# 0xSameer/ast

Measured on AMD Instinct MI355X. Metric: speech frames/s (train step), higher is better.
Workload: dtype f32 storage / f32 accumulate; batched GEMMs as bf16x3 splits on the bf16 MFMA pipe (every f32 operand value represented EXACTLY by three bf16 terms, f32 exponent range, six term products, each product exact to 2^-26: >= float32 on any data); the encoder recurrences multiply the same way (resident we

## Files before the change

### ast_amd/_lib.py

```python
import ctypes as C
import os

_HERE = os.path.dirname(os.path.abspath(__file__))
LIB_PATH = os.environ.get("ASTK_LIB_PATH") or os.path.join(_HERE, "libastk.so")

TEST_LIB_PATH = os.path.join(_HERE, "libastk_test.so")

MAX_CNN = 4
MAX_RNN = 8
MAX_ATTN = 4
PREC_DEFAULT, PREC_FP16X2, PREC_BF16X3, PREC_F32 = 0, 1, 2, 3
OPERANDS_DEFAULT, OPERANDS_F32, OPERANDS_FP16 = 0, 1, 2
OPERANDS_BY_NAME = {None: OPERANDS_DEFAULT, "default": OPERANDS_DEFAULT, "f32": OPERANDS_F32, "fp16": OPERANDS_FP16}
PREC_BY_NAME = {None: PREC_DEFAULT, "default": PREC_DEFAULT, "fp16x2": PREC_FP16X2, "bf16x3": PREC_BF16X3, "f32": PREC_F32}

c_float_p = C.POINTER(C.c_float)
c_int_p = C.POINTER(C.c_int32)
c_double_p = C.POINTER(C.c_double)


class _Sized:

    def __init__(self, *a, **k):
        super().__init__()
# ... 172 lines not shown
    "astk_persist_status_snapshot": (C.c_int, [_VP, _VP]),
    "astk_persist_status_merge": (C.c_int, [_VP, _VP]),
    "astk_persist_status": (C.c_int, [C.POINTER(C.c_uint), _I]),
    "astk_device_cu_count": (C.c_int, []),
    "astk_lstm_stack_path": (C.c_int, [C.POINTER(LstmStackDesc)]),
    "astk_lstm_stack_free_cus": (C.c_int, [C.POINTER(LstmStackDesc)]),
    "astk_decoder_path": (C.c_int, [C.POINTER(DecoderDesc)]),
    "astk_prof_begin": (C.c_int, []),
    "astk_prof_end": (C.c_int, [C.POINTER(C.c_double)]),
}

TEST_HOOK_SIGNATURES = {
    "astk_debug_set_amax_generation": (C.c_int, [C.c_uint]),
    "astk_conv_debug_preact": (C.c_int, [C.POINTER(CnnDesc), _VP, _SZ, _I, _VP, _VP]),
    "astk_conv_debug_kill_units": (C.c_int, [_VP, _I]),
    "astk_debug_gemm_group": (C.c_int, [_I, _I, c_int_p, c_int_p, c_int_p, C.POINTER(C.c_void_p), C.POINTER(C.c_void_p), C.POINTER(C.c_void_p), _I, _I, _VP]),
}

_lib = None
_test_lib = None


class AstkError(RuntimeError):
    pass


def load():
    global _lib
    if _lib is not None:
        return _lib
# ... 74 lines not shown
```

### ast_amd/csrc/common.h

```cpp
#pragma once
#include <hip/hip_runtime.h>
#include <stdint.h>
#include <stddef.h>
#include <stdio.h>
#include <string.h>
#include "../../include/astk.h"

namespace astk {

void set_error(const char* fmt, ...);

enum ProfCat { PROF_ATTN_FWD = 0, PROF_ATTN_BWD = 1, PROF_GEMM = 2, PROF_CELL = 3, PROF_DEC_FWD = 4, PROF_DEC_BWD = 5, PROF_NCAT = 6 };
bool prof_enabled();
float* prof_tick_buffer(int which);
void prof_start(int cat, hipStream_t s, double work);
void prof_stop(int cat, hipStream_t s);
void prof_add_bytes(int cat, double bytes);
struct ProfScope {
  int cat; hipStream_t s; bool on;
  ProfScope(int c, hipStream_t st, double work = 0.0) : cat(c), s(st), on(prof_enabled()) { if (on) prof_start(cat, s, work); }
  ~ProfScope() { if (on) prof_stop(cat, s); }
};

#define ASTK_CHECK(cond, ...)            \
// ... 36 lines not shown
enum PersistBit { PERSIST_ENC_FWD = 1, PERSIST_ENC_BWD = 2, PERSIST_DEC_FWD = 4, PERSIST_DEC_BWD = 8 };
struct AbortCtl {
  unsigned* word;
  unsigned* status;
  unsigned limit;
  unsigned bit;
};
AbortCtl abort_ctl(unsigned* word, unsigned bit);
int device_cu_count();
enum TuneKey {
  TUNE_GEMM_TILE, TUNE_GEMM_T256_ABOVE, TUNE_GEMM_GRID, TUNE_GEMM_HYBRID, TUNE_GEMM_CHUNK, TUNE_GEMM_CHUNK_DIV, TUNE_GEMM_LOG, TUNE_GEMM_TICKET,
  TUNE_GEMM_DETERMINISTIC, TUNE_GEMM_FORWARD_PAIRS,
  TUNE_CONV_DIRECT0, TUNE_CONV_SEQ_FWD, TUNE_CONV_SEQ_BWD, TUNE_CONV_SEQ_STATS_BLOCKS, TUNE_CONV_SEQ_APPLY_BLOCKS,
  TUNE_DEC_PERSIST, TUNE_DEC_B6_SPLIT, TUNE_DEC_B6_FUSED, TUNE_DEC_WIDE,
  TUNE_LSTM_PERSIST, TUNE_LSTM_HOIST, TUNE_LSTM_X3, TUNE_LSTM_X4, TUNE_LSTM_ROWS32, TUNE_LSTM_OVERLAP_CHUNK, TUNE_LSTM_SIDE_FWD, TUNE_LSTM_SIDE_BWD, TUNE_LSTM_DUO_SIDE,
  TUNE_ROW_LONGK, TUNE_PERSIST_SPIN_LIMIT, TUNE_COLREDUCE_BLOCKS,
  TUNE_COUNT
};
double tune(TuneKey k);
inline bool tune_on(TuneKey k) { return tune(k) != 0.0; }
__device__ __forceinline__ bool abort_seen(const AbortCtl& ab) {
  return __hip_atomic_load(ab.word, __ATOMIC_RELAXED, __HIP_MEMORY_SCOPE_AGENT) != 0;
}
__device__ __forceinline__ void abort_raise(const AbortCtl& ab) {
  __hip_atomic_store(ab.word, 1u, __ATOMIC_RELAXED, __HIP_MEMORY_SCOPE_AGENT);
  __hip_atomic_fetch_or(ab.status, ab.bit, __ATOMIC_RELAXED, __HIP_MEMORY_SCOPE_AGENT);
}

constexpr int AMAX_SLOT_WORDS = 16;
constexpr int AMAX_PSLOT_STRIDE = 16;
constexpr int AMAX_PSLOT_WORDS = AMAX_SLOT_WORDS * AMAX_PSLOT_STRIDE;
// ... 442 lines not shown
```

### ast_amd/csrc/conv.hip

```cpp
#include "common.h"
#include <atomic>
#include <mutex>
#include <algorithm>
#include <cstdlib>

namespace astk {

namespace {

struct CnnPlan {
  int n;
  int B, T, D;
  int Tn[ASTK_MAX_CNN_LAYERS], Fn[ASTK_MAX_CNN_LAYERS];
  int Tc[ASTK_MAX_CNN_LAYERS], Fc[ASTK_MAX_CNN_LAYERS];
  int pwt[ASTK_MAX_CNN_LAYERS], pwf[ASTK_MAX_CNN_LAYERS];
  bool pooled[ASTK_MAX_CNN_LAYERS];
  int Cn[ASTK_MAX_CNN_LAYERS];
  int rows[ASTK_MAX_CNN_LAYERS];
  int rowsc[ASTK_MAX_CNN_LAYERS];
  int K0, K0p;
  int JG, K0g, xf_rows;
  float* XF;
  int padA[ASTK_MAX_CNN_LAYERS];
  int dF[ASTK_MAX_CNN_LAYERS], dB[ASTK_MAX_CNN_LAYERS];
// ... 375 lines not shown
        }
        if (c + 16 < C) {
          *reinterpret_cast<float4*>(row + c + 16) = make_float4(sa[4], sa[5], sa[6], sa[7]);
          *reinterpret_cast<float4*>(row + C + c + 16) = make_float4(qa[4], qa[5], qa[6], qa[7]);
        }
      }
    }
  }
}
struct UnpackJobs {
  int n;
  const float* src[ASTK_MAX_CNN_LAYERS];
  float* dW[ASTK_MAX_CNN_LAYERS];
  int Co[ASTK_MAX_CNN_LAYERS], Ci[ASTK_MAX_CNN_LAYERS], KT[ASTK_MAX_CNN_LAYERS];
  int JG[ASTK_MAX_CNN_LAYERS], ldg[ASTK_MAX_CNN_LAYERS];
};
__global__ void k_unpack_dw(UnpackJobs jobs, const unsigned* __restrict__ status, float* __restrict__ status_dst) {
  const int q = blockIdx.y;
  if (status_dst && blockIdx.x == 0 && q == 0 && threadIdx.x == 0) *status_dst = (float)(*status);
  const float* const src = jobs.src[q];
  float* const dW = jobs.dW[q];
  const int Co = jobs.Co[q], Ci = jobs.Ci[q], KT = jobs.KT[q], JG = jobs.JG[q], ldg = jobs.ldg[q];
  const long n = (long)Co * Ci * KT;
  for (long i = blockIdx.x * (long)blockDim.x + threadIdx.x; i < n; i += (long)gridDim.x * blockDim.x) {
    if (ldg > 0) {
      const int j = (int)(i % Ci), t = (int)((i / Ci) % KT), c = (int)(i / ((long)Ci * KT));
      dW[i] += src[(long)c * ldg + t * JG + j];
    } else {
      const int k = (int)(i % KT), ci = (int)((i / KT) % Ci), co = (int)(i / ((long)Ci * KT));
      dW[i] += src[((long)co * KT + k) * Ci + ci];
    }
  }
}

__global__ __launch_bounds__(256) void k_repack_w(const float* __restrict__ W, float* __restrict__ Wr, int Co, int Ci, int KT, unsigned long long* amax,
                                                  const unsigned long long* fold_src, unsigned long long* fold_dst) {
  __shared__ float red4[4];
  if (fold_src && blockIdx.x == 0 && threadIdx.x < 64) amax_compact(fold_src, fold_dst);
  const long n = (long)Co * Ci * KT;
  float m = 0.f;
  for (long i = blockIdx.x * (long)blockDim.x + threadIdx.x; i < n; i += (long)gridDim.x * blockDim.x) {
    const int ci = (int)(i % Ci);
    const int k = (int)((i / Ci) % KT);
    const int co = (int)(i / ((long)Ci * KT));
    const float v = W[((long)co * Ci + ci) * KT + k];
    Wr[i] = v;
    m = fmaxf(m, fabsf(v));
  }
  if (amax) amax_emit_block(amax, m, red4);
}
struct PhaseWJobs {
  int n;
  float* wd[GEMM_GROUP_MAX];
  int r[GEMM_GROUP_MAX], na[GEMM_GROUP_MAX];
  unsigned long long* amax[GEMM_GROUP_MAX];
};
__global__ __launch_bounds__(256) void k_phase_w(const float* __restrict__ W, PhaseWJobs jobs, int Co, int Ci, int KT, int st,
                                                 const unsigned long long* fold_src, unsigned long long* fold_dst) {
  __shared__ float red4[4];
  if (fold_src && blockIdx.x == 0 && blockIdx.y == 0 && threadIdx.x < 64) amax_compact(fold_src, fold_dst);
  const int j = blockIdx.y, r = jobs.r[j], na = jobs.na[j];
  float* const Wd = jobs.wd[j];
  const long n = (long)Ci * na * Co;
  float m = 0.f;
  for (long i = blockIdx.x * (long)blockDim.x + threadIdx.x; i < n; i += (long)gridDim.x * blockDim.x) {
    const int co = (int)(i % Co);
    const int a = (int)((i / Co) % na);
    const int ci = (int)(i / ((long)Co * na));
    const int k = r + st * (na - 1 - a);
    const float v = W[((long)co * Ci + ci) * KT + k];
    Wd[i] = v;
    m = fmaxf(m, fabsf(v));
  }
  if (jobs.amax[j]) {
    amax_emit_block(jobs.amax[j], m, red4);
  }
}

__device__ __forceinline__ void colstats_finalize(int C, double* __restrict__ stat, const BnFinalize& fin);
__global__ __launch_bounds__(256) void k_colstats(const float* __restrict__ Y, int rows, int C, double* __restrict__ stat, BnFinalize fin) {
  colreduce_block<2>(
      rows, C,
      [&](int r, int c, float4* a) {
        const float4 v = *reinterpret_cast<const float4*>(Y + (long)r * C + c);
        a[0].x += v.x; a[0].y += v.y; a[0].z += v.z; a[0].w += v.w;
        a[1].x += v.x * v.x; a[1].y += v.y * v.y; a[1].z += v.z * v.z; a[1].w += v.w * v.w;
      },
      [&](int col, int st, float v) { atomicAdd(&stat[st * C + col], (double)v); });
  colstats_finalize(C, stat, fin);
}
// ... 586 lines not shown
int astk_conv_debug_preact(const astk_cnn_desc* d, void* ws, size_t ws_bytes, int layer, float* out, void* stream) {
  CnnPlan P;
  ASTK_TRY(make_plan(d, ws, P));
  ASTK_CHECK(ws && ws_bytes >= P.bytes && out && layer >= 0 && layer < P.n, "conv_debug_preact: bad arguments");
  const long n = (long)P.rows[layer] * P.Cn[layer];
  hipLaunchKernelGGL(k_preact, dim3(gridn((size_t)n)), dim3(256), 0, (hipStream_t)stream, P.Y[layer], P.bn[layer], out, n, P.Cn[layer]);
  ASTK_LAUNCH_CHECK();
  return 0;
}

int astk_conv_debug_kill_units(const int32_t* units, int n) {
  g_kill_units = n > 0 ? units : nullptr;
  g_kill_n = n > 0 && units ? n : 0;
  return 0;
}
#endif

int astk_conv_bn_relu_bwd(const astk_cnn_desc* d, const astk_cnn_layer_params* L, const astk_cnn_layer_grads* Gr, float* d_out,
                          void* ws, size_t ws_bytes, void* stream) {
  return astk_conv_bn_relu_bwd_sync(d, L, Gr, d_out, ws, ws_bytes, nullptr, nullptr, 1, stream);
}

int astk_conv_bn_relu_bwd_sync(const astk_cnn_desc* d, const astk_cnn_layer_params* L, const astk_cnn_layer_grads* Gr, float* d_out,
                               void* ws, size_t ws_bytes, astk_stat_exchange_fn exchange, void* user, int world, void* stream) {
  hipStream_t s = (hipStream_t)stream;
  ASTK_CHECK_DESC(d, astk_cnn_desc);
  PrecScope prec_scope(d->precision, d->gemm_operands);
  DetScope det_scope(d->deterministic);
  ASTK_CHECK(world >= 1, "conv_bn_relu_bwd: world %d", world);
  if (world == 1 || d->no_bn) exchange = nullptr;
// ... 9 lines not shown
  }
  const int B = P.B;
  const bool seq_off = !tune_on(TUNE_CONV_SEQ_BWD);
  bool seq_last = !seq_off && seq_bwd_applicable(P.Cn[P.n - 1], P.Fn[P.n - 1], (long)P.Tn[P.n - 1] * B);
#ifdef ASTK_TEST_HOOKS
  if (g_kill_n > 0) seq_last = false;
#endif
  if (!seq_last) {
    const int i = P.n - 1;
    const size_t shm = (size_t)P.Cn[i] * P.Fn[i] * sizeof(float);
    hipLaunchKernelGGL(k_seq_to_rows, dim3(P.Tn[i], B), dim3(256), shm, s, d_out, P.G, B, P.Fn[i], P.Tn[i], P.Cn[i]);
    ASTK_LAUNCH_CHECK();
  }
  UnpackJobs uj;
  uj.n = 0;
  size_t uj_max = 0;
  auto unpack_add = [&](const float* src, float* dW, int Co, int Ci, int KT, int JG, int ldg) {
    uj.src[uj.n] = src; uj.dW[uj.n] = dW; uj.Co[uj.n] = Co; uj.Ci[uj.n] = Ci; uj.KT[uj.n] = KT; uj.JG[uj.n] = JG; uj.ldg[uj.n] = ldg;
    ++uj.n;
    uj_max = std::max(uj_max, (size_t)Co * Ci * KT);
  };
  for (int i = P.n - 1; i >= 0; --i) {
    const int C = P.Cn[i], rows = P.rows[i];
#ifdef ASTK_TEST_HOOKS
    if (g_kill_n > 0) {
      hipLaunchKernelGGL(k_kill_units, dim3(cdiv(g_kill_n, 256)), dim3(256), 0, s, P.G, g_kill_units, g_kill_n, i, rows, C);
      ASTK_LAUNCH_CHECK();
    }
#endif
    if (i == P.n - 1 && !conv_take_bwd_clean(ws)) ASTK_TRY(fill_zero(P.stat[0], P.zero_bwd_bytes, s));
    const bool seq = seq_last && i == P.n - 1;
    const int seq_gx = C / SEQ_CH;
    if (seq) {
      const int sb = (int)tune(TUNE_CONV_SEQ_STATS_BLOCKS);
      const int gy = std::max(1, std::min(sb / seq_gx, cdiv(P.Tn[i] * B, seq_pp(P.Fn[i]))));
// ... 46 lines not shown
        unpack_add(P.dWr[0], Gr[0].dW, C, d->kf[0], d->kt[0], P.JG, ldg);
      } else {
      ASTK_TRY(gemm_launch(GEMM_TN, gemm_args(C, P.K0p, P.rowsc[0], mat(P.DY[0], C), mat(P.P0, P.K0p), P.dWr[0], P.K0p, nullptr, GEMM_ATOMIC, ks), s));
      ASTK_TRY(add2d_f32(Gr[0].dW, P.K0, P.dWr[0], P.K0p, C, P.K0, s));
      }
    } else {
      const int Ci = P.Cn[i - 1], KT = d->kt[i], st = d->st[i], pt = d->pt[i];
      const long dyrow = (long)Tp * C;
      const long hprow = (long)(P.Tn[i - 1] + 2 * P.padA[i - 1]) * Ci;
      const unsigned long long* ady = P.a_dy[i];
      GemmArgs ph[GEMM_GROUP_MAX];
      int nph = 0;
      bool folded = false;
      PhaseWJobs pj;
      pj.n = 0;
      int pj_na_max = 0;
      auto launch_phase_w = [&]() {
        if (pj.n == 0) return;
        hipLaunchKernelGGL(k_phase_w, dim3(gridn((size_t)Ci * pj_na_max * C / 8), pj.n), dim3(256), 0, s, L[i].W, pj, C, Ci, KT, st,
                           folded ? nullptr : (const unsigned long long*)P.a_dy_s[i], P.a_dy[i]);
        folded = true;
        pj.n = 0;
        pj_na_max = 0;
      };
      for (int rho = 0; rho < st && rho < P.Tn[i - 1]; ++rho) {
        const int r = (rho + pt) % st;
        const int na = (KT - r + st - 1) / st;
        if (na <= 0) {
          continue;
        }
        const int nj = (P.Tn[i - 1] - rho + st - 1) / st;
        const int q0 = (rho + pt) / st;
        if (nph == P.wd_copies) {
          launch_phase_w();
          ASTK_LAUNCH_CHECK();
          ASTK_TRY(gemm_launch_group(GEMM_NT, ph, nph, s));
          nph = 0;
        }
        float* wd = P.Wd + (size_t)nph * P.wd_stride;
        pj.wd[pj.n] = wd; pj.r[pj.n] = r; pj.na[pj.n] = na; pj.amax[pj.n] = P.a_wd[nph];
        ++pj.n;
        pj_na_max = std::max(pj_na_max, na);
        const long start = (long)(q0 - na + 1 + P.dF[i]);
        ASTK_CHECK(start >= 0, "cnn dgrad: negative window start");
        GemmArgs g = gemm_args(B * F * nj, Ci, na * C, mat2(P.DY[i] + start * C, nj, dyrow, C), mat(wd, (long)na * C),
                               P.G + (long)rho * Ci, Ci);
        g.c_tn = nj;
        g.c_sg = (long)P.Tn[i - 1] * Ci;
        g.c_st = (long)st * Ci;
        ph[nph] = with_amax_b(with_amax_a(lowp(g), ady), P.a_wd[nph]);
        ++nph;
      }
      launch_phase_w();
      ASTK_LAUNCH_CHECK();
      if (!folded) ady = P.a_dy_s[i];
      {
        MatView A = mat2(P.DY[i] + (long)P.dF[i] * C, P.Tc[i], dyrow, C);
        MatView Bm = mat2(P.HP[i - 1], P.Tc[i], hprow, (long)st * Ci);
        const long tiles = (long)cdiv(C, 128) * cdiv(KT * Ci, 128);
        ASTK_TRY(gemm_launch(GEMM_TN, with_amax_b(with_amax_a(lowp(gemm_args(C, KT * Ci, P.rowsc[i], A, Bm, P.dWr[i], (long)KT * Ci, nullptr, GEMM_ATOMIC, ksplit_for(tiles, P.rowsc[i]))), ady), P.a_hp[i - 1]), s));
      }
      unpack_add(P.dWr[i], Gr[i].dW, C, Ci, KT, 0, 0);
      if (nph > 0) ASTK_TRY(gemm_launch_group(GEMM_NT, ph, nph, s));
    }
  }
  if (uj.n > 0) {
    hipLaunchKernelGGL(k_unpack_dw, dim3(gridn(uj_max), uj.n), dim3(256), 0, s, uj, persist_status_word(), d->status_dst);
    ASTK_LAUNCH_CHECK();
  } else if (d->status_dst) {
    ASTK_TRY(status_snapshot_launch(d->status_dst, s));
  }
  return 0;
}

}
```

### ast_amd/csrc/decoder.hip

```cpp
#include "common.h"
#include <mutex>
#include "decoder_wide.h"

namespace astk {

constexpr int PDEC_MAX_LAYERS = 3;
struct DecPersistBuffers {
  int32_t *TOK, *PRED;
  float *X0, *Q, *ALPHA, *CVH, *HT, *LOGITS, *LOSSROWS;
  float *G[PDEC_MAX_LAYERS], *C[PDEC_MAX_LAYERS], *HR[PDEC_MAX_LAYERS], *HD[PDEC_MAX_LAYERS];
  float *LSE, *PART, *CESTAT, *ENCA, *ML;
  unsigned* ctr;
  void* zero_a; size_t zero_a_bytes; void* zero_b; size_t zero_b_bytes;
  const float *c0, *h0;
};
bool decoder_persist_applicable(const astk_decoder_desc* d, int* nsplit_out, int* chunk_out);
int decoder_persist_fwd_launch(const astk_decoder_desc* d, const astk_decoder_params* prm, const float* enc, const int32_t* y,
                               const int32_t* ytgt, const int32_t* use_truth, const float* emb_mask, const float* rnn_masks, const DecPersistBuffers& bf,
                               float* loss, int32_t* pred_out, hipStream_t s);

struct DecPersistBwdBuffers {
  void* zero_ptr; size_t zero_bytes;
  void* zero2_ptr; size_t zero2_bytes;
  const float *WoT, *WcT, *ENCA, *CVH, *HT, *LOGITS, *ML;
// ... 263 lines not shown
  if (threadIdx.x == 0) *dst = (float)(red[0] + red[1] + red[2] + red[3]);
}

__global__ void k_copy_i32(int32_t* dst, const int32_t* src, int n) {
  const int i = blockIdx.x * blockDim.x + threadIdx.x;
  if (i < n) dst[i] = src[i];
}

__global__ void k_dtanh_inplace(float* __restrict__ x, const float* __restrict__ y, long n) {
  for (long i = blockIdx.x * (long)blockDim.x + threadIdx.x; i < n; i += (long)gridDim.x * blockDim.x) {
    const float t = y[i];
    x[i] *= 1.f - t * t;
  }
}

RowGemmArgs rg(int M, int N, const float* A, long lda, const float* W, long ldw, int K, float* out, long ld_out) {
  RowGemmArgs a;
  memset(&a, 0, sizeof(a));
  a.npairs = 1;
  a.p[0].A = A; a.p[0].lda = lda; a.p[0].W = W; a.p[0].ldw = ldw; a.p[0].K = K;
  a.M = M; a.N = N; a.out = out; a.ld_out = ld_out;
  return a;
}

int ksplit_rows(long tiles, int rows) {
  long s = 256 / (tiles > 0 ? tiles : 1);
  if (s < 1) s = 1;
  long smax = rows / 128;
  if (smax < 1) smax = 1;
  return (int)(s > smax ? smax : s);
// ... 374 lines not shown
  {
    TransposeJobs tj;
    tj.n = 0;
    if (persist) transpose_add(tj, P.WoT, Vp, prm->Wo, A, V, A);
    transpose_add(tj, P.WcT, A, prm->Wc, CW, A, CW);
    for (int k = 0; k < NA; ++k) transpose_add(tj, P.WaT + (size_t)k * H * H, H, k == 0 ? prm->Wa : prm->Wa_x[k - 1], H, H, H);
    for (int l = 0; l < nl; ++l) {
      const int in = l == 0 ? XI : H;
      if (tj.n + 2 > FILL_SEG_MAX) { ASTK_TRY(transpose_batch(tj, s)); tj.n = 0; }
      transpose_add(tj, P.WuT[l], 4 * H, prm->lstm[l].Wu, in, 4 * H, in);
      transpose_add(tj, P.WlT[l], 4 * H, prm->lstm[l].Wl, H, 4 * H, H);
    }
    ASTK_TRY(transpose_batch(tj, s));
  }
  if (!persist) ASTK_TRY(attn_ws_init(P.attn_ws, B, T, H, s));
  if (persist) {
    DecPersistBwdBuffers bf;
    memset(&bf, 0, sizeof(bf));
    bf.WoT = P.WoT; bf.WcT = P.WcT; bf.ENCA = P.ENCA; bf.ALPHA = P.ALPHA; bf.CVH = P.CVH; bf.ML = P.MLB;
    for (int l = 0; l < nl; ++l) { bf.WlT[l] = P.WlT[l]; bf.WuT[l] = P.WuT[l]; bf.C[l] = P.C[l]; bf.G[l] = P.G[l]; }
    bf.HT = P.HT; bf.LOGITS = P.LOGITS; bf.DPRE = P.DPRE; bf.DCVH = P.DCVH; bf.DS = P.DS; bf.DX0 = P.DX0;
    bf.DHATT = P.PART; bf.d_c0 = d_c0; bf.ctr = P.PCTR;
    bf.DXH = b6s ? P.DXH : nullptr;
    bf.zero_ptr = d->zero_ptr; bf.zero_bytes = d->zero_bytes;
    bf.zero2_ptr = d_enc; bf.zero2_bytes = (size_t)B * T * H * sizeof(float);
    ASTK_TRY(decoder_persist_bwd_launch(d, enc, rnn_masks, bf, s));
  }
  if (!persist) {
    ASTK_TRY(gemm_launch(GEMM_NN, gemm_args(S * B, A, V, mat(P.LOGITS, Vp), mat(prm->Wo, A), P.DPRE, A), s));
    const long r0 = P.feed ? (long)(S - 1) * B * A : 0, n = (long)S * B * A - r0;
    hipLaunchKernelGGL(k_dtanh_inplace, dim3((unsigned)std::min<long>(cdiv(n, 256), 2048)), dim3(256), 0, s, P.DPRE + r0, P.HT + (size_t)B * A + r0, n);
    ASTK_LAUNCH_CHECK();
  }
  if (wide_b) {
    DecWideBwdBuffers wb;
    wb.WcT = P.WcT; wb.WaT = P.WaT; wb.WlT = P.WlT[0]; wb.WuT = P.WuT[0]; wb.ALPHA = P.ALPHA; wb.CVH = P.CVH; wb.HT = P.HT; wb.C = P.C[0];
    wb.G = P.G[0]; wb.DPRE = P.DPRE; wb.DCVH = P.DCVH; wb.DS = P.DS; wb.DQ = P.DQ; wb.DHTOP = P.DHTOP; wb.DC0 = P.DC[0][0];
    wb.scratch = P.WBWD; wb.ctr = P.WBCTR;
    ASTK_TRY(decoder_wide_bwd_launch(d, enc, rnn_masks, wb, s));
  }
// ... 60 lines not shown
    }
    {
      RowGemmArgs a = rg(B, XI, P.G[0] + (size_t)st * B * 4 * H, 4 * H, P.WuT[0], 4 * H, 4 * H, P.DX0 + (size_t)st * B * XI, XI);
      if (P.feed && st > 0) {
        a.carry = P.DPRE + (size_t)(st - 1) * B * A; a.ld_carry = A;
        a.carry_aux = P.HT + (size_t)st * B * A; a.ld_carry_aux = A;
        a.carry_col0 = E;
      }
      ASTK_TRY(rowgemm_launch(a, s));
    }
  }
  for (int l = 0; l < nl; ++l) {
    ASTK_TRY(rowgemm_launch(rg(B, H, P.G[l], 4 * H, P.WlT[l], 4 * H, 4 * H, d_h0 + l * bh, H), s));
    if (!persist) ASTK_TRY(copy_f32(d_c0 + l * bh, P.DC[l][0], bh, s));
  }
  if (persist && 2 * NA <= GEMM_GROUP_MAX) {
    GemmArgs list[GEMM_GROUP_MAX];
    int n = 0;
    for (int k = 0; k < NA; ++k) {
      GemmArgs ga = gemm_args(T, H, S, mat(P.ALPHA + (size_t)k * S * B * Tp, (long)B * Tp), mat(P.DCVH + (size_t)k * H, (long)B * CW), d_enc, H, nullptr, GEMM_ATOMIC);
      ga.batch = B; ga.sA = Tp; ga.sB = CW; ga.sC = (long)T * H;
      list[n++] = ga;
      GemmArgs gb = gemm_args(T, H, S, mat(P.DS + (size_t)k * S * B * Tp, (long)B * Tp), mat(P.Q + (size_t)k * S * bh, (long)B * H), d_enc, H, nullptr, GEMM_ATOMIC);
      gb.batch = B; gb.sA = Tp; gb.sB = H; gb.sC = (long)T * H;
      list[n++] = gb;
    }
    ASTK_TRY(gemm_launch_group(GEMM_TN, list, n, s));
  } else
  for (int k = 0; k < NA; ++k) {
    GemmArgs ga = gemm_args(T, H, S, mat(P.ALPHA + (size_t)k * S * B * Tp, (long)B * Tp), mat(P.DCVH + (size_t)k * H, (long)B * CW), d_enc, H, nullptr,
                            k == 0 ? GEMM_STORE : GEMM_ACCUM);
// ... 181 lines not shown
```

### ast_amd/csrc/util.hip

```cpp
#include "common.h"
#include <algorithm>
#include <stdarg.h>
#include <vector>
#include <atomic>
#include <mutex>

namespace astk {

static thread_local char g_err[512] = "";

void set_error(const char* fmt, ...) {
  va_list ap;
  va_start(ap, fmt);
  vsnprintf(g_err, sizeof(g_err), fmt, ap);
  va_end(ap);
}
const char* last_error() { return g_err; }

struct ProfState {
  bool on = false;
  std::vector<hipEvent_t> ev[PROF_NCAT];
  double work[PROF_NCAT] = {0, 0, 0, 0, 0, 0};
  double bytes[PROF_NCAT] = {0, 0, 0, 0, 0, 0};
};
// ... 61 lines not shown
    {TUNE_DEC_B6_SPLIT, "dec.b6_split", 1},
    {TUNE_DEC_B6_FUSED, "dec.b6_fused", 1},
    {TUNE_DEC_WIDE, "dec.wide", 1},
    {TUNE_LSTM_PERSIST, "lstm.persist", 1},
    {TUNE_LSTM_HOIST, "lstm.hoist", 1},
    {TUNE_LSTM_X3, "lstm.x3", 1},
    {TUNE_LSTM_X4, "lstm.x4", 1},
    {TUNE_LSTM_ROWS32, "lstm.rows32", -1},
    {TUNE_LSTM_OVERLAP_CHUNK, "lstm.overlap_chunk", 0},
    {TUNE_LSTM_SIDE_FWD, "lstm.side_fwd", 1},
    {TUNE_LSTM_SIDE_BWD, "lstm.side_bwd", 0},
    {TUNE_LSTM_DUO_SIDE, "lstm.duo_side", 0},
    {TUNE_ROW_LONGK, "row.longk", 2048},
    {TUNE_PERSIST_SPIN_LIMIT, "persist.spin_limit", 0},
    {TUNE_COLREDUCE_BLOCKS, "colreduce.blocks", 256},
};
constexpr bool tune_table_in_order() {
  for (int i = 0; i < TUNE_COUNT; ++i)
    if (g_tune_table[i].key != i) return false;
  return true;
}
static_assert(tune_table_in_order(), "g_tune_table rows must follow enum TuneKey");
static std::atomic<double> g_tune[TUNE_COUNT];
static std::atomic<int> g_tune_init{0};
static void tune_init() {
  if (g_tune_init.load(std::memory_order_acquire)) return;
  static std::mutex mu;
  std::lock_guard<std::mutex> lock(mu);
  if (g_tune_init.load()) return;
  for (int i = 0; i < TUNE_COUNT; ++i) g_tune[i].store(g_tune_table[i].def);
// ... 64 lines not shown
__global__ void k_transpose(float* dst, long ldd, const float* src, long lds, int rows, int cols) {
  __shared__ float t[32][33];
  const int bx = blockIdx.x * 32, by = blockIdx.y * 32;
  const int tx = threadIdx.x & 31, ty = threadIdx.x >> 5;
  for (int j = ty; j < 32; j += 8) {
    const int r = by + j, c = bx + tx;
    t[j][tx] = (r < rows && c < cols) ? src[(long)r * lds + c] : 0.f;
  }
  __syncthreads();
  for (int j = ty; j < 32; j += 8) {
    const int c = bx + j, r = by + tx;
    if (c < cols && r < ldd) dst[(long)c * ldd + r] = t[tx][j];
  }
}

__global__ void k_transpose_batch(TransposeJobs tj) {
  const int job = blockIdx.z;
  const int rows = tj.rows[job], cols = tj.cols[job];
  const long ldd = tj.ldd[job], lds = tj.lds[job];
  const int bx = blockIdx.x * 32, by = blockIdx.y * 32;
  if (bx >= cols || by >= ldd) return;
  __shared__ float t[32][33];
  const float* src = tj.src[job];
  float* dst = tj.dst[job];
  const int tx = threadIdx.x & 31, ty = threadIdx.x >> 5;
  for (int j = ty; j < 32; j += 8) {
    const int r = by + j, c = bx + tx;
    t[j][tx] = (r < rows && c < cols) ? src[(long)r * lds + c] : 0.f;
  }
  __syncthreads();
  for (int j = ty; j < 32; j += 8) {
    const int c = bx + j, r = by + tx;
    if (c < cols && r < ldd) dst[(long)c * ldd + r] = t[tx][j];
  }
}

__global__ __launch_bounds__(256) void k_copy_segments(CopySegs cs) {
  const int seg = blockIdx.y;
  const size_t n16 = cs.bytes[seg] / 16;
  const uint4* src = reinterpret_cast<const uint4*>(cs.src[seg]);
  uint4* dst = reinterpret_cast<uint4*>(cs.dst[seg]);
  for (size_t i = blockIdx.x * (size_t)blockDim.x + threadIdx.x; i < n16; i += (size_t)gridDim.x * blockDim.x) dst[i] = src[i];
  if (blockIdx.x == 0) {
    const unsigned* sw = reinterpret_cast<const unsigned*>(cs.src[seg]);
    unsigned* dw = reinterpret_cast<unsigned*>(cs.dst[seg]);
    for (size_t i = n16 * 4 + threadIdx.x; i < cs.bytes[seg] / 4; i += blockDim.x) dw[i] = sw[i];
  }
}
// ... 291 lines not shown
int axpy_rows(float* dst, const float* src, size_t n, hipStream_t s) {
  if (n == 0) return 0;
  hipLaunchKernelGGL(k_axpy, dim3(grid_for(n)), dim3(256), 0, s, dst, src, n);
  ASTK_LAUNCH_CHECK();
  return 0;
}
int transpose_f32(float* dst, long ldd, const float* src, long lds, int rows, int cols, hipStream_t s) {
  if (rows <= 0 || cols <= 0) return 0;
  hipLaunchKernelGGL(k_transpose, dim3(cdiv(cols, 32), cdiv(ldd, 32)), dim3(256), 0, s, dst, ldd, src, lds, rows, cols);
  ASTK_LAUNCH_CHECK();
  return 0;
}
int transpose_batch(const TransposeJobs& t, hipStream_t s) {
  if (t.n <= 0) return 0;
  int gx = 1, gy = 1;
  for (int i = 0; i < t.n; ++i) { gx = std::max(gx, cdiv(t.cols[i], 32)); gy = std::max(gy, cdiv(t.ldd[i], 32)); }
  hipLaunchKernelGGL(k_transpose_batch, dim3(gx, gy, t.n), dim3(256), 0, s, t);
  ASTK_LAUNCH_CHECK();
  return 0;
}
int copy_segments(const CopySegs& c, hipStream_t s) {
  if (c.n <= 0) return 0;
  size_t mx = 0;
  for (int i = 0; i < c.n; ++i) {
    ASTK_CHECK(aligned16(c.dst[i]) && aligned16(c.src[i]) && (c.bytes[i] % 4) == 0, "copy_segments: segment %d must be 16-byte aligned, size a multiple of 4", i);
    mx = std::max(mx, c.bytes[i]);
  }
  unsigned gx = (unsigned)((mx / 16 + 256 * 4 - 1) / (256 * 4));
  gx = gx < 1 ? 1 : (gx > 512 ? 512 : gx);
  hipLaunchKernelGGL(k_copy_segments, dim3(gx, (unsigned)c.n), dim3(256), 0, s, c);
  ASTK_LAUNCH_CHECK();
// ... 323 lines not shown
```

### include/astk.h

```cpp
#ifndef ASTK_H
#define ASTK_H
#include <stddef.h>
#include <stdint.h>

#ifdef __cplusplus
extern "C" {
#endif

#define ASTK_VERSION 107
#define ASTK_MAX_CNN_LAYERS 4
#define ASTK_MAX_RNN_LAYERS 8
#define ASTK_MAX_ATTN 4

int astk_version(void);
const char* astk_last_error(void);

enum { ASTK_PREC_DEFAULT = 0, ASTK_PREC_FP16X2 = 1, ASTK_PREC_BF16X3 = 2, ASTK_PREC_F32 = 3 };
enum { ASTK_OPERANDS_DEFAULT = 0, ASTK_OPERANDS_F32 = 1, ASTK_OPERANDS_FP16 = 2 };

int astk_gemm_f32(int layout, int M, int N, int K,
                  const float* A, long lda, const float* B, long ldb, float* C, long ldc,
                  const float* bias, int mode, int ksplit, int batch, long sA, long sB, long sC, void* stream);
int astk_gemm_f32_ex(int layout, int M, int N, int K,
                     const float* A, long lda, const float* B, long ldb, float* C, long ldc,
// ... 46 lines not shown
  float* dbeta;
  float* dbias;
} astk_cnn_layer_grads;

int astk_conv_bn_relu_out_dims(const astk_cnn_desc* d, int* T_out, int* F_out, int* feat_dim);
size_t astk_conv_bn_relu_workspace_bytes(const astk_cnn_desc* d);
int astk_conv_bn_relu_fwd(const astk_cnn_desc* d, const astk_cnn_layer_params* layers, const float* X,
                          const float* noise, float* out, void* ws, size_t ws_bytes, int train, void* stream);
int astk_conv_bn_relu_bwd(const astk_cnn_desc* d, const astk_cnn_layer_params* layers,
                          const astk_cnn_layer_grads* grads, float* d_out, void* ws, size_t ws_bytes, void* stream);
const void* astk_conv_out_amax(const astk_cnn_desc* d, void* ws, size_t ws_bytes);

#ifdef ASTK_TEST_HOOKS
int astk_conv_debug_preact(const astk_cnn_desc* d, void* ws, size_t ws_bytes, int layer, float* out, void* stream);
int astk_conv_debug_kill_units(const int32_t* units, int n);
#endif

typedef int (*astk_stat_exchange_fn)(void* user, double* stat, int n, void* stream);
int astk_conv_bn_relu_fwd_sync(const astk_cnn_desc* d, const astk_cnn_layer_params* layers, const float* X, const float* noise,
                               float* out, void* ws, size_t ws_bytes, int train, astk_stat_exchange_fn exchange, void* user,
                               int world, void* stream);
int astk_conv_bn_relu_bwd_sync(const astk_cnn_desc* d, const astk_cnn_layer_params* layers, const astk_cnn_layer_grads* grads,
                               float* d_out, void* ws, size_t ws_bytes, astk_stat_exchange_fn exchange, void* user, int world,
                               void* stream);

typedef struct {
  size_t struct_size;
  int T, B, in_dim, h, n_layers, n_dirs;
  float out_bound;
  const void* x_amax;
// ... 223 lines not shown
```

Measured before the change: 4.653 million.

## Tile conv weight re-layouts through shared memory and compute d_enc directly

Rewrites the conv dW unpack and phase-weight re-layout kernels to stage slabs in shared memory, so reads and writes are coalesced and vectorised instead of strided. The phase kernel now handles all phases in one pass over a weight tile. Widens the batched transpose to 64x64 tiles with float4 accesses. Adds a fused decoder kernel that builds d_enc from the attention weights, their gradients, the context rows and Q, replacing a grouped GEMM and a zero-fill; it is on by default behind a tune flag. The trade-off is larger shared-memory footprints and a scalar-FMA path standing in for the MFMA GEMM.

```diff
diff --git a/ast_amd/_lib.py b/ast_amd/_lib.py
--- a/ast_amd/_lib.py
+++ b/ast_amd/_lib.py
@@ -210,6 +210,11 @@
     "astk_debug_set_amax_generation": (C.c_int, [C.c_uint]),
     "astk_conv_debug_preact": (C.c_int, [C.POINTER(CnnDesc), _VP, _SZ, _I, _VP, _VP]),
     "astk_conv_debug_kill_units": (C.c_int, [_VP, _I]),
+    "astk_conv_debug_repack_w": (C.c_int, [_VP, _VP, _I, _I, _I, _VP, _VP]),
+    "astk_conv_debug_phase_w": (C.c_int, [_VP, _I, C.POINTER(C.c_void_p), c_int_p, c_int_p, C.POINTER(C.c_void_p), _I, _I, _I, _I, _VP]),
+    "astk_conv_debug_unpack_dw": (C.c_int, [_VP, _VP, _I, _I, _I, _VP]),
+    "astk_conv_debug_transpose_batch": (C.c_int, [_I, C.POINTER(C.c_void_p), C.POINTER(C.c_long), C.POINTER(C.c_void_p), C.POINTER(C.c_long),
+                                                  c_int_p, c_int_p, _VP]),
     "astk_debug_gemm_group": (C.c_int, [_I, _I, c_int_p, c_int_p, c_int_p, C.POINTER(C.c_void_p), C.POINTER(C.c_void_p), C.POINTER(C.c_void_p), _I, _I, _VP]),
 }
 
diff --git a/ast_amd/csrc/common.h b/ast_amd/csrc/common.h
--- a/ast_amd/csrc/common.h
+++ b/ast_amd/csrc/common.h
@@ -74,7 +74,7 @@
   TUNE_CONV_DIRECT0, TUNE_CONV_SEQ_FWD, TUNE_CONV_SEQ_BWD, TUNE_CONV_SEQ_STATS_BLOCKS, TUNE_CONV_SEQ_APPLY_BLOCKS,
   TUNE_DEC_PERSIST, TUNE_DEC_B6_SPLIT, TUNE_DEC_B6_FUSED, TUNE_DEC_WIDE,
   TUNE_LSTM_PERSIST, TUNE_LSTM_HOIST, TUNE_LSTM_X3, TUNE_LSTM_X4, TUNE_LSTM_ROWS32, TUNE_LSTM_OVERLAP_CHUNK, TUNE_LSTM_SIDE_FWD, TUNE_LSTM_SIDE_BWD, TUNE_LSTM_DUO_SIDE,
-  TUNE_ROW_LONGK, TUNE_PERSIST_SPIN_LIMIT, TUNE_COLREDUCE_BLOCKS,
+  TUNE_ROW_LONGK, TUNE_PERSIST_SPIN_LIMIT, TUNE_COLREDUCE_BLOCKS, TUNE_DEC_DENC_DIRECT,
   TUNE_COUNT
 };
 double tune(TuneKey k);
diff --git a/ast_amd/csrc/conv.hip b/ast_amd/csrc/conv.hip
--- a/ast_amd/csrc/conv.hip
+++ b/ast_amd/csrc/conv.hip
@@ -413,22 +413,60 @@
   float* dW[ASTK_MAX_CNN_LAYERS];
   int Co[ASTK_MAX_CNN_LAYERS], Ci[ASTK_MAX_CNN_LAYERS], KT[ASTK_MAX_CNN_LAYERS];
   int JG[ASTK_MAX_CNN_LAYERS], ldg[ASTK_MAX_CNN_LAYERS];
+  int cb[ASTK_MAX_CNN_LAYERS];
 };
+template <class F>
+__device__ __forceinline__ void seg_load(const float* __restrict__ p, int n, int lane, int nl, F f) {
+  const int head = min(n, (int)((16u - ((unsigned)(uintptr_t)p & 15u)) & 15u) >> 2), nv = (n - head) >> 2, tail = head + 4 * nv;
+  for (int i = lane; i < head; i += nl) f(i, p[i]);
+  for (int v = lane; v < nv; v += nl) {
+    const int i = head + 4 * v;
+    const float4 x = *reinterpret_cast<const float4*>(p + i);
+    f(i, x.x); f(i + 1, x.y); f(i + 2, x.z); f(i + 3, x.w);
+  }
+  for (int i = tail + lane; i < n; i += nl) f(i, p[i]);
+}
+template <class G>
+__device__ __forceinline__ void seg_update(float* __restrict__ p, int n, int lane, int nl, G g) {
+  const int head = min(n, (int)((16u - ((unsigned)(uintptr_t)p & 15u)) & 15u) >> 2), nv = (n - head) >> 2, tail = head + 4 * nv;
+  for (int i = lane; i < head; i += nl) p[i] = g(i, p[i]);
+  for (int v = lane; v < nv; v += nl) {
+    const int i = head + 4 * v;
+    float4 x = *reinterpret_cast<float4*>(p + i);
+    x.x = g(i, x.x); x.y = g(i + 1, x.y); x.z = g(i + 2, x.z); x.w = g(i + 3, x.w);
+    *reinterpret_cast<float4*>(p + i) = x;
+  }
+  for (int i = tail + lane; i < n; i += nl) p[i] = g(i, p[i]);
+}
+static inline int slab_cb(int Ci, int KT) {
+  int cb = 64;
+  while (cb > 4 && (long)cb * KT > 2048) cb >>= 1;
+  return std::min(cb, Ci);
+}
 __global__ void k_unpack_dw(UnpackJobs jobs, const unsigned* __restrict__ status, float* __restrict__ status_dst) {
+  extern __shared__ float slab[];
   const int q = blockIdx.y;
   if (status_dst && blockIdx.x == 0 && q == 0 && threadIdx.x == 0) *status_dst = (float)(*status);
   const float* const src = jobs.src[q];
   float* const dW = jobs.dW[q];
   const int Co = jobs.Co[q], Ci = jobs.Ci[q], KT = jobs.KT[q], JG = jobs.JG[q], ldg = jobs.ldg[q];
-  const long n = (long)Co * Ci * KT;
-  for (long i = blockIdx.x * (long)blockDim.x + threadIdx.x; i < n; i += (long)gridDim.x * blockDim.x) {
-    if (ldg > 0) {
+  if (ldg > 0) {
+    const long n = (long)Co * Ci * KT;
+    for (long i = blockIdx.x * (long)blockDim.x + threadIdx.x; i < n; i += (long)gridDim.x * blockDim.x) {
       const int j = (int)(i % Ci), t = (int)((i / Ci) % KT), c = (int)(i / ((long)Ci * KT));
       dW[i] += src[(long)c * ldg + t * JG + j];
-    } else {
-      const int k = (int)(i % KT), ci = (int)((i / KT) % Ci), co = (int)(i / ((long)Ci * KT));
-      dW[i] += src[((long)co * KT + k) * Ci + ci];
-    }
+    }
+    return;
+  }
+  const int cb = jobs.cb[q], nb = (Ci + cb - 1) / cb;
+  const int lane = threadIdx.x & 31, sub = threadIdx.x >> 5, nsub = blockDim.x >> 5;
+  for (long u = blockIdx.x; u < (long)Co * nb; u += gridDim.x) {
+    const int co = (int)(u / nb), ci0 = (int)(u % nb) * cb, w = min(cb, Ci - ci0);
+    for (int k = sub; k < KT; k += nsub)
+      seg_load(src + ((long)co * KT + k) * Ci + ci0, w, lane, 32, [&](int c, float v) { slab[c * KT + k] = v; });
+    __syncthreads();
+    seg_update(dW + ((long)co * Ci + ci0) * KT, w * KT, threadIdx.x, blockDim.x, [&](int i, float old) { return old + slab[i]; });
+    __syncthreads();
   }
 }
 
@@ -454,25 +492,36 @@
   int r[GEMM_GROUP_MAX], na[GEMM_GROUP_MAX];
   unsigned long long* amax[GEMM_GROUP_MAX];
 };
-__global__ __launch_bounds__(256) void k_phase_w(const float* __restrict__ W, PhaseWJobs jobs, int Co, int Ci, int KT, int st,
+constexpr int PW_CO = 64;
+static inline int phase_cib(int Ci, int KT) { return std::max(1, std::min(std::min(8, Ci), 80 / KT)); }
+__global__ __launch_bounds__(256) void k_phase_w(const float* __restrict__ W, PhaseWJobs jobs, int Co, int Ci, int KT, int st, int cib,
                                                  const unsigned long long* fold_src, unsigned long long* fold_dst) {
+  extern __shared__ float slab[];
   __shared__ float red4[4];
-  if (fold_src && blockIdx.x == 0 && blockIdx.y == 0 && threadIdx.x < 64) amax_compact(fold_src, fold_dst);
-  const int j = blockIdx.y, r = jobs.r[j], na = jobs.na[j];
-  float* const Wd = jobs.wd[j];
-  const long n = (long)Ci * na * Co;
-  float m = 0.f;
-  for (long i = blockIdx.x * (long)blockDim.x + threadIdx.x; i < n; i += (long)gridDim.x * blockDim.x) {
-    const int co = (int)(i % Co);
-    const int a = (int)((i / Co) % na);
-    const int ci = (int)(i / ((long)Co * na));
-    const int k = r + st * (na - 1 - a);
-    const float v = W[((long)co * Ci + ci) * KT + k];
-    Wd[i] = v;
-    m = fmaxf(m, fabsf(v));
-  }
-  if (jobs.amax[j]) {
-    amax_emit_block(jobs.amax[j], m, red4);
+  if (fold_src && blockIdx.x == 0 && threadIdx.x < 64) amax_compact(fold_src, fold_dst);
+  const int ncb = (Ci + cib - 1) / cib;
+  const int co0 = (int)(blockIdx.x / ncb) * PW_CO, ci0 = (int)(blockIdx.x % ncb) * cib;
+  const int cow = min(PW_CO, Co - co0), ciw = min(cib, Ci - ci0), pitch = cib * KT + 1;
+  const int lane = threadIdx.x & 15, sub = threadIdx.x >> 4;
+  for (int c = sub; c < cow; c += 16)
+    seg_load(W + ((long)(co0 + c) * Ci + ci0) * KT, ciw * KT, lane, 16, [&](int i, float v) { slab[c * pitch + i] = v; });
+  __syncthreads();
+  for (int j = 0; j < jobs.n; ++j) {
+    const int r = jobs.r[j], na = jobs.na[j];
+    float* const Wd = jobs.wd[j];
+    float m = 0.f;
+    for (int sg = sub; sg < ciw * na; sg += 16) {
+      const int c = sg / na, a = sg % na, k = r + st * (na - 1 - a);
+      seg_update(Wd + ((long)(ci0 + c) * na + a) * Co + co0, cow, lane, 16, [&](int o, float) {
+        const float v = slab[o * pitch + c * KT + k];
+        m = fmaxf(m, fabsf(v));
+        return v;
+      });
+    }
+    if (jobs.amax[j]) {
+      amax_emit_block(jobs.amax[j], m, red4);
+      __syncthreads();
+    }
   }
 }
 
@@ -1089,6 +1138,49 @@
   g_kill_n = n > 0 && units ? n : 0;
   return 0;
 }
+
+int astk_conv_debug_repack_w(const float* W, float* Wr, int Co, int Ci, int KT, unsigned long long* amax, void* stream) {
+  ASTK_CHECK(W && Wr && Co > 0 && Ci > 0 && KT > 0, "conv_debug_repack_w: bad arguments");
+  hipLaunchKernelGGL(k_repack_w, dim3(gridn((size_t)Co * Ci * KT / 8)), dim3(256), 0, (hipStream_t)stream, W, Wr, Co, Ci, KT, amax, nullptr, nullptr);
+  ASTK_LAUNCH_CHECK();
+  return 0;
+}
+int astk_conv_debug_phase_w(const float* W, int n, float* const* wd, const int* r, const int* na, unsigned long long* const* amax, int Co, int Ci,
+                            int KT, int st, void* stream) {
+  ASTK_CHECK(W && wd && r && na && n > 0 && n <= GEMM_GROUP_MAX && Co > 0 && Ci > 0 && KT > 0 && KT <= 160 && st > 0, "conv_debug_phase_w: bad arguments");
+  PhaseWJobs pj;
+  pj.n = n;
+  for (int j = 0; j < n; ++j) {
+    ASTK_CHECK(na[j] > 0 && r[j] >= 0 && r[j] + st * (na[j] - 1) < KT, "conv_debug_phase_w: phase %d reaches past the kernel", j);
+    pj.wd[j] = wd[j]; pj.r[j] = r[j]; pj.na[j] = na[j]; pj.amax[j] = amax ? amax[j] : nullptr;
+  }
+  const int cib = phase_cib(Ci, KT);
+  hipLaunchKernelGGL(k_phase_w, dim3((unsigned)(cdiv(Co, PW_CO) * cdiv(Ci, cib))), dim3(256), (size_t)PW_CO * (cib * KT + 1) * sizeof(float),
+                     (hipStream_t)stream, W, pj, Co, Ci, KT, st, cib, nullptr, nullptr);
+  ASTK_LAUNCH_CHECK();
+  return 0;
+}
+int astk_conv_debug_unpack_dw(const float* dWr, float* dW, int Co, int Ci, int KT, void* stream) {
+  ASTK_CHECK(dWr && dW && Co > 0 && Ci > 0 && KT > 0 && KT <= 160, "conv_debug_unpack_dw: bad arguments");
+  UnpackJobs uj;
+  uj.n = 1;
+  uj.src[0] = dWr; uj.dW[0] = dW; uj.Co[0] = Co; uj.Ci[0] = Ci; uj.KT[0] = KT; uj.JG[0] = 0; uj.ldg[0] = 0; uj.cb[0] = slab_cb(Ci, KT);
+  hipLaunchKernelGGL(k_unpack_dw, dim3((unsigned)std::min<long>((long)Co * cdiv(Ci, uj.cb[0]), 4096), 1), dim3(256),
+                     (size_t)uj.cb[0] * KT * sizeof(float), (hipStream_t)stream, uj, persist_status_word(), nullptr);
+  ASTK_LAUNCH_CHECK();
+  return 0;
+}
+int astk_conv_debug_transpose_batch(int n, float* const* dst, const long* ldd, const float* const* src, const long* lds, const int* rows,
+                                    const int* cols, void* stream) {
+  ASTK_CHECK(n > 0 && n <= FILL_SEG_MAX && dst && ldd && src && lds && rows && cols, "conv_debug_transpose_batch: bad arguments");
+  TransposeJobs tj;
+  tj.n = 0;
+  for (int j = 0; j < n; ++j) {
+    ASTK_CHECK(ldd[j] >= rows[j] && lds[j] >= cols[j], "conv_debug_transpose_batch: job %d: pitch below extent", j);
+    transpose_add(tj, dst[j], ldd[j], src[j], lds[j], rows[j], cols[j]);
+  }
+  return transpose_batch(tj, (hipStream_t)stream);
+}
 #endif
 
 int astk_conv_bn_relu_bwd(const astk_cnn_desc* d, const astk_cnn_layer_params* L, const astk_cnn_layer_grads* Gr, float* d_out,
@@ -1128,11 +1220,13 @@
   }
   UnpackJobs uj;
   uj.n = 0;
-  size_t uj_max = 0;
+  size_t uj_max = 0, uj_shm = 0;
   auto unpack_add = [&](const float* src, float* dW, int Co, int Ci, int KT, int JG, int ldg) {
     uj.src[uj.n] = src; uj.dW[uj.n] = dW; uj.Co[uj.n] = Co; uj.Ci[uj.n] = Ci; uj.KT[uj.n] = KT; uj.JG[uj.n] = JG; uj.ldg[uj.n] = ldg;
+    uj.cb[uj.n] = ldg > 0 ? 0 : slab_cb(Ci, KT);
+    uj_max = std::max(uj_max, ldg > 0 ? (size_t)gridn((size_t)Co * Ci * KT) : (size_t)Co * cdiv(Ci, uj.cb[uj.n]));
+    uj_shm = std::max(uj_shm, (size_t)uj.cb[uj.n] * KT * sizeof(float));
     ++uj.n;
-    uj_max = std::max(uj_max, (size_t)Co * Ci * KT);
   };
   for (int i = P.n - 1; i >= 0; --i) {
     const int C = P.Cn[i], rows = P.rows[i];
@@ -1209,14 +1303,14 @@
       bool folded = false;
       PhaseWJobs pj;
       pj.n = 0;
-      int pj_na_max = 0;
+      ASTK_CHECK(KT <= 160, "conv_bn_relu_bwd: kernel extent %d of layer %d does not fit the re-layout tiles", KT, i);
       auto launch_phase_w = [&]() {
         if (pj.n == 0) return;
-        hipLaunchKernelGGL(k_phase_w, dim3(gridn((size_t)Ci * pj_na_max * C / 8), pj.n), dim3(256), 0, s, L[i].W, pj, C, Ci, KT, st,
-                           folded ? nullptr : (const unsigned long long*)P.a_dy_s[i], P.a_dy[i]);
+        const int cib = phase_cib(Ci, KT);
+        hipLaunchKernelGGL(k_phase_w, dim3((unsigned)(cdiv(C, PW_CO) * cdiv(Ci, cib))), dim3(256), (size_t)PW_CO * (cib * KT + 1) * sizeof(float), s,
+                           L[i].W, pj, C, Ci, KT, st, cib, folded ? nullptr : (const unsigned long long*)P.a_dy_s[i], P.a_dy[i]);
         folded = true;
         pj.n = 0;
-        pj_na_max = 0;
       };
       for (int rho = 0; rho < st && rho < P.Tn[i - 1]; ++rho) {
         const int r = (rho + pt) % st;
@@ -1235,7 +1329,6 @@
         float* wd = P.Wd + (size_t)nph * P.wd_stride;
         pj.wd[pj.n] = wd; pj.r[pj.n] = r; pj.na[pj.n] = na; pj.amax[pj.n] = P.a_wd[nph];
         ++pj.n;
-        pj_na_max = std::max(pj_na_max, na);
         const long start = (long)(q0 - na + 1 + P.dF[i]);
         ASTK_CHECK(start >= 0, "cnn dgrad: negative window start");
         GemmArgs g = gemm_args(B * F * nj, Ci, na * C, mat2(P.DY[i] + start * C, nj, dyrow, C), mat(wd, (long)na * C),
@@ -1260,7 +1353,7 @@
     }
   }
   if (uj.n > 0) {
-    hipLaunchKernelGGL(k_unpack_dw, dim3(gridn(uj_max), uj.n), dim3(256), 0, s, uj, persist_status_word(), d->status_dst);
+    hipLaunchKernelGGL(k_unpack_dw, dim3((unsigned)std::min<size_t>(uj_max, 4096), uj.n), dim3(256), uj_shm, s, uj, persist_status_word(), d->status_dst);
     ASTK_LAUNCH_CHECK();
   } else if (d->status_dst) {
     ASTK_TRY(status_snapshot_launch(d->status_dst, s));
diff --git a/ast_amd/csrc/decoder.hip b/ast_amd/csrc/decoder.hip
--- a/ast_amd/csrc/decoder.hip
+++ b/ast_amd/csrc/decoder.hip
@@ -301,6 +301,57 @@
   }
 }
 
+constexpr int DE_TT = 16, DE_HT = 256, DE_SC = 64;
+__global__ __launch_bounds__(256) void k_denc_direct(const float* __restrict__ ALPHA, const float* __restrict__ DS, const float* __restrict__ DCVH,
+                                                     const float* __restrict__ Q, float* __restrict__ d_enc, int B, int S, int T, int Tp, int H,
+                                                     int CW, int NA) {
+  __shared__ __attribute__((aligned(16))) float la[DE_SC][DE_TT];
+  __shared__ __attribute__((aligned(16))) float ld[DE_SC][DE_TT];
+  const int b = blockIdx.x, t0 = blockIdx.y * DE_TT, h = blockIdx.z * DE_HT + 4 * (threadIdx.x & 63), r0 = 4 * (threadIdx.x >> 6);
+  const bool live = h < H;
+  float4 acc[4];
+#pragma unroll
+  for (int r = 0; r < 4; ++r) acc[r] = make_float4(0.f, 0.f, 0.f, 0.f);
+  for (int k = 0; k < NA; ++k) {
+    for (int s0 = 0; s0 < S; s0 += DE_SC) {
+      const int sc = min(DE_SC, S - s0);
+      __syncthreads();
+      for (int i = threadIdx.x; i < sc * DE_TT; i += 256) {
+        const int sl = i / DE_TT, r = i % DE_TT, t = t0 + r;
+        const size_t off = (((size_t)k * S + s0 + sl) * B + b) * Tp + t;
+        la[sl][r] = t < T ? ALPHA[off] : 0.f;
+        ld[sl][r] = t < T ? DS[off] : 0.f;
+      }
+      __syncthreads();
+      if (live) {
+        const float* pc = DCVH + ((size_t)s0 * B + b) * CW + (size_t)k * H + h;
+        const float* pq = Q + (((size_t)k * S + s0) * B + b) * H + h;
+#pragma unroll 8
+        for (int sl = 0; sl < sc; ++sl) {
+          const float4 c = *reinterpret_cast<const float4*>(pc), q = *reinterpret_cast<const float4*>(pq);
+          pc += (size_t)B * CW;
+          pq += (size_t)B * H;
+          const float4 a0 = *reinterpret_cast<const float4*>(&la[sl][r0]), d0 = *reinterpret_cast<const float4*>(&ld[sl][r0]);
+          const float av[4] = {a0.x, a0.y, a0.z, a0.w}, dv[4] = {d0.x, d0.y, d0.z, d0.w};
+#pragma unroll
+          for (int r = 0; r < 4; ++r) {
+            acc[r].x = fmaf(av[r], c.x, acc[r].x); acc[r].y = fmaf(av[r], c.y, acc[r].y);
+            acc[r].z = fmaf(av[r], c.z, acc[r].z); acc[r].w = fmaf(av[r], c.w, acc[r].w);
+            acc[r].x = fmaf(dv[r], q.x, acc[r].x); acc[r].y = fmaf(dv[r], q.y, acc[r].y);
+            acc[r].z = fmaf(dv[r], q.z, acc[r].z); acc[r].w = fmaf(dv[r], q.w, acc[r].w);
+          }
+        }
+      }
+    }
+  }
+  if (!live) return;
+#pragma unroll
+  for (int r = 0; r < 4; ++r) {
+    const int t = t0 + r0 + r;
+    if (t < T) *reinterpret_cast<float4*>(d_enc + ((size_t)b * T + t) * H + h) = acc[r];
+  }
+}
+
 RowGemmArgs rg(int M, int N, const float* A, long lda, const float* W, long ldw, int K, float* out, long ld_out) {
   RowGemmArgs a;
   memset(&a, 0, sizeof(a));
@@ -705,6 +756,7 @@
     ASTK_TRY(transpose_batch(tj, s));
   }
   if (!persist) ASTK_TRY(attn_ws_init(P.attn_ws, B, T, H, s));
+  const bool denc_direct = persist && tune_on(TUNE_DEC_DENC_DIRECT) && H % 4 == 0 && CW % 4 == 0 && aligned16(d_enc);
   if (persist) {
     DecPersistBwdBuffers bf;
     memset(&bf, 0, sizeof(bf));
@@ -714,7 +766,7 @@
     bf.DHATT = P.PART; bf.d_c0 = d_c0; bf.ctr = P.PCTR;
     bf.DXH = b6s ? P.DXH : nullptr;
     bf.zero_ptr = d->zero_ptr; bf.zero_bytes = d->zero_bytes;
-    bf.zero2_ptr = d_enc; bf.zero2_bytes = (size_t)B * T * H * sizeof(float);
+    if (!denc_direct) { bf.zero2_ptr = d_enc; bf.zero2_bytes = (size_t)B * T * H * sizeof(float); }
     ASTK_TRY(decoder_persist_bwd_launch(d, enc, rnn_masks, bf, s));
   }
   if (!persist) {
@@ -805,7 +857,10 @@
     ASTK_TRY(rowgemm_launch(rg(B, H, P.G[l], 4 * H, P.WlT[l], 4 * H, 4 * H, d_h0 + l * bh, H), s));
     if (!persist) ASTK_TRY(copy_f32(d_c0 + l * bh, P.DC[l][0], bh, s));
   }
-  if (persist && 2 * NA <= GEMM_GROUP_MAX) {
+  if (denc_direct) {
+    hipLaunchKernelGGL(k_denc_direct, dim3(B, cdiv(T, DE_TT), cdiv(H, DE_HT)), dim3(256), 0, s, P.ALPHA, P.DS, P.DCVH, P.Q, d_enc, B, S, T, Tp, H, CW, NA);
+    ASTK_LAUNCH_CHECK();
+  } else if (persist && 2 * NA <= GEMM_GROUP_MAX) {
     GemmArgs list[GEMM_GROUP_MAX];
     int n = 0;
     for (int k = 0; k < NA; ++k) {
diff --git a/ast_amd/csrc/util.hip b/ast_amd/csrc/util.hip
--- a/ast_amd/csrc/util.hip
+++ b/ast_amd/csrc/util.hip
@@ -99,6 +99,7 @@
     {TUNE_ROW_LONGK, "row.longk", 2048},
     {TUNE_PERSIST_SPIN_LIMIT, "persist.spin_limit", 0},
     {TUNE_COLREDUCE_BLOCKS, "colreduce.blocks", 256},
+    {TUNE_DEC_DENC_DIRECT, "dec.denc_direct", 1},
 };
 constexpr bool tune_table_in_order() {
   for (int i = 0; i < TUNE_COUNT; ++i)
@@ -193,24 +194,45 @@
   }
 }
 
-__global__ void k_transpose_batch(TransposeJobs tj) {
+__global__ __launch_bounds__(256) void k_transpose_batch(TransposeJobs tj) {
   const int job = blockIdx.z;
   const int rows = tj.rows[job], cols = tj.cols[job];
   const long ldd = tj.ldd[job], lds = tj.lds[job];
-  const int bx = blockIdx.x * 32, by = blockIdx.y * 32;
+  const int bx = blockIdx.x * 64, by = blockIdx.y * 64;
   if (bx >= cols || by >= ldd) return;
-  __shared__ float t[32][33];
+  __shared__ float t[64][65];
   const float* src = tj.src[job];
   float* dst = tj.dst[job];
-  const int tx = threadIdx.x & 31, ty = threadIdx.x >> 5;
-  for (int j = ty; j < 32; j += 8) {
-    const int r = by + j, c = bx + tx;
-    t[j][tx] = (r < rows && c < cols) ? src[(long)r * lds + c] : 0.f;
+  const bool vsrc = (((uintptr_t)src & 15) | (lds & 3)) == 0, vdst = (((uintptr_t)dst & 15) | (ldd & 3)) == 0;
+  const int q = (threadIdx.x & 15) * 4, ty = threadIdx.x >> 4;
+  for (int j = ty; j < 64; j += 16) {
+    const int r = by + j, c = bx + q;
+    float4 v = make_float4(0.f, 0.f, 0.f, 0.f);
+    if (r < rows) {
+      const float* p = src + (long)r * lds + c;
+      if (vsrc && c + 3 < cols) v = *reinterpret_cast<const float4*>(p);
+      else {
+        if (c < cols) v.x = p[0];
+        if (c + 1 < cols) v.y = p[1];
+        if (c + 2 < cols) v.z = p[2];
+        if (c + 3 < cols) v.w = p[3];
+      }
+    }
+    t[j][q] = v.x; t[j][q + 1] = v.y; t[j][q + 2] = v.z; t[j][q + 3] = v.w;
   }
   __syncthreads();
-  for (int j = ty; j < 32; j += 8) {
-    const int c = bx + j, r = by + tx;
-    if (c < cols && r < ldd) dst[(long)c * ldd + r] = t[tx][j];
+  for (int j = ty; j < 64; j += 16) {
+    const int c = bx + j, r = by + q;
+    if (c >= cols || r >= ldd) continue;
+    float* p = dst + (long)c * ldd + r;
+    const float4 v = make_float4(t[q][j], t[q + 1][j], t[q + 2][j], t[q + 3][j]);
+    if (vdst && r + 3 < ldd) *reinterpret_cast<float4*>(p) = v;
+    else {
+      p[0] = v.x;
+      if (r + 1 < ldd) p[1] = v.y;
+      if (r + 2 < ldd) p[2] = v.z;
+      if (r + 3 < ldd) p[3] = v.w;
+    }
   }
 }
 
@@ -532,7 +554,7 @@
 int transpose_batch(const TransposeJobs& t, hipStream_t s) {
   if (t.n <= 0) return 0;
   int gx = 1, gy = 1;
-  for (int i = 0; i < t.n; ++i) { gx = std::max(gx, cdiv(t.cols[i], 32)); gy = std::max(gy, cdiv(t.ldd[i], 32)); }
+  for (int i = 0; i < t.n; ++i) { gx = std::max(gx, cdiv(t.cols[i], 64)); gy = std::max(gy, cdiv(t.ldd[i], 64)); }
   hipLaunchKernelGGL(k_transpose_batch, dim3(gx, gy, t.n), dim3(256), 0, s, t);
   ASTK_LAUNCH_CHECK();
   return 0;
diff --git a/include/astk.h b/include/astk.h
--- a/include/astk.h
+++ b/include/astk.h
@@ -84,6 +84,12 @@
 #ifdef ASTK_TEST_HOOKS
 int astk_conv_debug_preact(const astk_cnn_desc* d, void* ws, size_t ws_bytes, int layer, float* out, void* stream);
 int astk_conv_debug_kill_units(const int32_t* units, int n);
+int astk_conv_debug_repack_w(const float* W, float* Wr, int Co, int Ci, int KT, unsigned long long* amax, void* stream);
+int astk_conv_debug_phase_w(const float* W, int n, float* const* wd, const int* r, const int* na, unsigned long long* const* amax, int Co, int Ci,
+                            int KT, int st, void* stream);
+int astk_conv_debug_unpack_dw(const float* dWr, float* dW, int Co, int Ci, int KT, void* stream);
+int astk_conv_debug_transpose_batch(int n, float* const* dst, const long* ldd, const float* const* src, const long* lds, const int* rows,
+                                    const int* cols, void* stream);
 #endif
 
 typedef int (*astk_stat_exchange_fn)(void* user, double* stat, int n, void* stream);
```

Result: no change. 4.659 million, median of 6 (+0.1%).
